# CTPLab/Tera-MIND

Hardware: AMD Instinct MI355X
Metric: denoising steps/sec on 64x64x(2 stains x 2 z) patches (interior patch-steps/s) (higher is better)
Workload: dtype f32; 1 GPU; configs[1]: b=32 images x 1 interior 64x64 patch (P=1, 128 padded + 32 collage patches/step), rna_slc=4, rna_num=229, stain=all, DDPM T=50 schedule, f32, mode A (pad+patchify -> UNet -> DDPM update); parallelism=dp1 (independent patch batches)

## Files before the change

tera-mind_amd/csrc/tm_kernels.hip:

```cpp
#include "tm_conv_pair.h"

#include <stdlib.h>
#include <string.h>

#include <type_traits>

namespace tmk {

template <int NZI, int WM, int TW, bool UPS = false>
struct C3Geo {
  static constexpr int TW_ = TW;
  static constexpr int MV = 4 * WM * 32;
  static constexpr int TR = (MV / TW < TW) ? (MV / TW) : TW;
  static constexpr int NPB = MV / (TR * TW);
  static constexpr int HR = TR + 2, HC = TW + 2;
  static constexpr int XV = NPB * NZI * HR * HC;
  static constexpr int XPIECES = XV * 2;
  static constexpr int PX = (XPIECES + 255) / 256;
  static constexpr int TZ = UPS ? 4 : 9;
  static constexpr int NTAP = TZ * NZI;
  static constexpr int WFLOATS = NTAP * 512;
  static constexpr int WPIECES = WFLOATS / 4;
  static constexpr int PW = (WPIECES + 255) / 256;
  static constexpr int TAPS_TOTAL = (NZI == 1) ? 9 : 3 * TZ;
// ... 518 lines not shown
  const f32x4 zero4 = {0.f, 0.f, 0.f, 0.f};
  auto load_x = [&](int cb) {
    const float* xp = a.x + (long)cb * a.x_plane;
#pragma unroll
    for (int z = 0; z < 2; ++z) {
      const float* b = xp + xoff + z * zplane;
      xr[z][0] = okl ? *(const f32x4*)(b - 8) : zero4;
      xr[z][1] = xoff >= 0 ? *(const f32x4*)(b) : zero4;
      xr[z][2] = xoff >= 0 ? *(const f32x4*)(b + 8) : zero4;
      xr[z][3] = okr ? *(const f32x4*)(b + 16) : zero4;
    }
  };
  auto put_t = [&](int p, const f32x4& d0, const f32x4& d1, const f32x4& d2, const f32x4& d3) __attribute__((always_inline)) {
    float* d = lds + xw + p * 4 * G::XP * 8;
    *(f32x4*)(d) = d0 - d2;
    *(f32x4*)(d + G::XP * 8) = d1 + d2;
    *(f32x4*)(d + 2 * G::XP * 8) = d2 - d1;
    *(f32x4*)(d + 3 * G::XP * 8) = d1 - d3;
  };

  load_x(0);
#pragma unroll
  for (int k = 0; k < G::KP; ++k) issue_piece(0, k);
  auto stage = [&](int cb, auto more_c) __attribute__((always_inline)) {
    constexpr bool more = decltype(more_c)::value;
    asm volatile("s_waitcnt vmcnt(0)" ::: "memory");
    __builtin_amdgcn_s_barrier();
    asm volatile("" ::: "memory");
    if (tid < G::XITEMS) {
      put_t(2, xr[0][0], xr[0][1], xr[0][2], xr[0][3]);
#pragma unroll
      for (int c = 0; c < 4; ++c) xr[0][c] = xr[0][c] + xr[1][c];
      put_t(0, xr[0][0], xr[0][1], xr[0][2], xr[0][3]);
      put_t(1, xr[1][0], xr[1][1], xr[1][2], xr[1][3]);
    }
    __builtin_amdgcn_s_waitcnt(0xC07F);
    asm volatile("" ::: "memory");
    __builtin_amdgcn_s_barrier();
    asm volatile("" ::: "memory");
    __builtin_amdgcn_sched_barrier(0);
    if (more) load_x(cb + 1);

    __builtin_amdgcn_s_setprio(1);
#pragma unroll
    for (int p = 0; p < 3; ++p) {
      const int n = cb * 3 + p;
      if (p > 0) {
        asm volatile("s_waitcnt vmcnt(0)" ::: "memory");
        __builtin_amdgcn_sched_barrier(0);
        __builtin_amdgcn_s_barrier();
        asm volatile("" ::: "memory");
        __builtin_amdgcn_sched_barrier(0);
      }
      const float* lwc = lw + (n & 1) * G::WSLOT + wb;
#pragma unroll
      for (int ky = 0; ky < 3; ++ky) {
#pragma unroll
        for (int q = 0; q < G::NQ; ++q) {
          const int tap = ky * 4 + q;
          const f32x4 wf = *(const f32x4*)(lwc + tap * 512);
          const f32x4 xf = ((const f32x4*)lds)[xb + xp_xtap<G>(p, q, ky) / 4];
#pragma unroll
          for (int kk = 0; kk < 4; ++kk) acc[p][q] = __builtin_amdgcn_mfma_f32_32x32x2f32(wf[kk], xf[kk], acc[p][q], 0, 0, 0);
          if (ky * G::NQ + q < G::KP && (p < 2 || more)) issue_piece(n + 1, ky * G::NQ + q);
        }
      }
    }
    __builtin_amdgcn_s_setprio(0);
  };
  for (int cb = 0; cb + 1 < a.Cbi; ++cb) stage(cb, std::true_type{});
  stage(a.Cbi - 1, std::false_type{});
  const int nte = 2 * nt + ch;
  if constexpr (HALF) {
    const int qh = __builtin_amdgcn_readfirstlane(wv >> 1);
    __syncthreads();
    auto hand_over = [&](const f32x16& t, int p) __attribute__((always_inline)) {
#pragma unroll
      for (int i = 0; i < 4; ++i) {
        const f32x4 v = {t[4 * i], t[4 * i + 1], t[4 * i + 2], t[4 * i + 3]};
        *(f32x4*)(lds + ((wv * 3 + p) * 4 + i) * 256 + lane * 4) = v;
      }
    };
    if (qh) {
#pragma unroll
      for (int p = 0; p < 3; ++p) hand_over(acc[p][0], p);
    } else {
#pragma unroll
      for (int p = 0; p < 3; ++p) hand_over(acc[p][1], p);
    }
    __syncthreads();
    f32x16 got[3];
#pragma unroll
    for (int p = 0; p < 3; ++p)
#pragma unroll
      for (int i = 0; i < 4; ++i) {
        const f32x4 v = *(const f32x4*)(lds + (((wv ^ 2) * 3 + p) * 4 + i) * 256 + lane * 4);
#pragma unroll
        for (int e = 0; e < 4; ++e) got[p][4 * i + e] = v[e];
      }
#pragma unroll
    for (int p = 0; p < 3; ++p) {
      acc[p][0] = qh ? (got[p] - acc[p][0]) - acc[p][1] : (acc[p][0] + acc[p][1]) + got[p];
      asm volatile("" : "+v"(acc[p][0]));
    }
#pragma unroll
    for (int z = 0; z < 2; ++z) {
      f32x16 o[1][1];
      o[0][0] = acc[0][0] + acc[1 + z][0];
      asm volatile("" : "+v"(o[0][0]));
      const int ooff[1] = {ooff0 >= 0 ? ooff0 + (z * S * S + qh) * 8 : -1};
      __builtin_amdgcn_sched_barrier(0);
      conv_epilogue<1, 1>(a, o, nte, h, on, ooff, 2 * S);
    }
  } else {
#pragma unroll
    for (int p = 0; p < 3; ++p) {
      const f32x16 ev = (acc[p][0] + acc[p][1]) + acc[p][2];
      acc[p][1] = (acc[p][1] - acc[p][2]) - acc[p][3];
      acc[p][0] = ev;
      asm volatile("" : "+v"(acc[p][0]), "+v"(acc[p][1]));
    }
#pragma unroll
    for (int z = 0; z < 2; ++z)
#pragma unroll
      for (int par = 0; par < 2; ++par) {
        f32x16 o[1][1];
        o[0][0] = acc[0][par] + acc[1 + z][par];
        asm volatile("" : "+v"(o[0][0]));
        const int ooff[1] = {ooff0 >= 0 ? ooff0 + (z * S * S + par) * 8 : -1};
        __builtin_amdgcn_sched_barrier(0);
        conv_epilogue<1, 1>(a, o, nte, h, on, ooff, 2 * S);
      }
  }
}

template <int HALF, int TW, int PIPE = 0>
struct XQGeo {
  static constexpr int TW_ = TW;
  static constexpr int NW = HALF ? 4 : 8;
  static constexpr int MG = 16 * NW;
  static constexpr int GW = TW / 4;
  static constexpr int TR = (MG / GW < TW) ? (MG / GW) : TW;
  static constexpr int NPB = MG / (TR * GW);
  static constexpr int HR = TR + 2;
  static constexpr int XP = NPB * HR * GW;
  static constexpr int XITEMS = XP * 2;
  static_assert(XP % 8 == 0, "whole groups of eight staging items (tm_conv_frag.h)");
  static constexpr int WTAP = 256;
  static constexpr int WSLOT = 18 * WTAP;
  static constexpr int KP = (18 + NW - 1) / NW;
  static constexpr int XSET = 6 * XP * 8;
  static constexpr int NSET = PIPE ? 2 : 3;
  static constexpr int XCH = NW * 3 * 1024;
  static constexpr int LDS_BYTES = (2 * WSLOT + NSET * XSET > XCH ? 2 * WSLOT + NSET * XSET : XCH) * 4;
  static_assert(2 * WSLOT * 4 <= 65536 && LDS_BYTES <= 160 * 1024, "LDS-DMA destinations below 64 KiB, the CU's LDS");
  static_assert(!PIPE || !HALF || LDS_BYTES <= 80 * 1024, "two workgroups of the small tile per CU");
};
template <class V>
TM_HD V xq_transform(int q, const V (&d)[6]) {
  switch (q) {
    case 0: return (4.f * d[0] - 5.f * d[2]) + d[4];
    case 1: return (d[3] + d[4]) - 4.f * (d[1] + d[2]);
    case 2: return 4.f * (d[1] - d[2]) - (d[3] - d[4]);
    case 3: return 2.f * (d[3] - d[1]) + (d[4] - d[2]);
    case 4: return 2.f * (d[1] - d[3]) + (d[4] - d[2]);
    default: return (4.f * d[1] - 5.f * d[3]) + d[5];
  }
}
TM_HD constexpr int xq_lane_group(int tw, int i32) { return tw == 8 ? conv_lane_voxel(16, i32) : i32; }
template <class G>
TM_HD constexpr int xq_xtap(int q, int ky) { return q * G::XP * 8 + conv_frag_off(ky * G::GW, 0, G::XP); }
template <class G>
TM_HD constexpr int xq_xfrag(int set, int qh, int lxb) { return set * G::XSET + 3 * qh * G::XP * 8 + lxb; }
template <class G>
TM_HD constexpr int xq_xstage(int set, int q, int item) {
  return set * G::XSET + q * G::XP * 8 + conv_frag_off(conv_stage_row(item), conv_stage_half(item), G::XP);
}

template <int HALF, int TW, int PIPE>
__global__ __launch_bounds__(HALF ? 256 : 512, 2) void conv3d_xquad(ConvArgs a) {
  using G = XQGeo<HALF, TW, PIPE>;
  static_assert(G::XITEMS <= 64 * G::NW, "one staging item per thread");
  extern __shared__ __attribute__((aligned(16))) float lds[];
  float* lw = lds;

  const int tid = threadIdx.x;
  const int lane = tid & 63, wv = tid >> 6;
  const int i32 = lane & 31, h = lane >> 5;

  const int S = a.S;
  const ConvTile t = conv_tile_of<TW, G::TR, false, false>(a);
  const int nt = t.nt, pg = t.pg, tr = t.tr, tc = t.tc;

  long xoff = -1;
  bool okl = false, okr = false;
  if (tid < G::XITEMS) {
    const int half = conv_stage_half(tid);
    int v = conv_stage_row(tid);
    const int j = v % G::GW; v /= G::GW;
    const int hr = v % G::HR;
    const int ps = v / G::HR;
    const int n = pg * G::NPB + ps;
    const int y = tr * G::TR + hr - 1, x = tc * TW + 4 * j;
    if (n < a.N && y >= 0 && y < S) {
      xoff = (long)n * a.x_nstride + ((long)y * S + x) * 8 + half * 4;
      okl = x > 0;
      okr = x + 4 < S;
    }
  }
  const long zplane = (long)S * S * 8;
  int xw = 2 * G::WSLOT + xq_xstage<G>(0, 0, tid);
  asm volatile("" : "+v"(xw));

  const int gt = wv >> 1;
  const int qh = wv & 1;
  int xb[3], on[1], ooff0;
  {
    const ConvLane l = conv_lane_of<G::TR, G::GW, G::HR * G::GW, G::GW, G::XP>(gt * 32 + xq_lane_group(TW, i32), h, 0, 0);
#pragma unroll
    for (int p = 0; p < 3; ++p) {
      xb[p] = (2 * G::WSLOT + xq_xfrag<G>(p, qh, l.xb)) / 4;
      asm volatile("" : "+v"(xb[p]));
    }
    const int n = pg * G::NPB + l.ps;
    on[0] = n;
    const int y = tr * G::TR + l.r, x = tc * TW + 4 * l.c;
    ooff0 = n < a.N ? (y * S + x) * 8 : -1;
  }
  const int wb = 3 * qh * G::WTAP + conv_frag_off(i32, h, 32);

  f32x16 acc[3][3];
  clear_acc(acc);

  const unsigned lw_lds = (unsigned)(size_t)(__attribute__((address_space(3))) float*)lw;
  const rsrc_words wrs = weight_rsrc<true>(a.w + (long)nt * a.Cbi * 3 * G::WSLOT, a.Cbi * 3 * G::WSLOT * 4);
  const int wvo = lane * 16;
  const int wvu = __builtin_amdgcn_readfirstlane(wv);
  auto issue_piece = [&](int n, int k) __attribute__((always_inline)) {
    lds_dma_piece<4, 18, G::NW>(lw_lds, (n & 1) * G::WSLOT, n * G::WSLOT, k, wvu, wvo, wrs);
  };

  f32x4 xr[2][6];
  const f32x4 zero4 = {0.f, 0.f, 0.f, 0.f};
  auto load_x = [&](int cb) {
    const float* xp = a.x + (long)cb * a.x_plane;
#pragma unroll
    for (int z = 0; z < 2; ++z) {
      const float* b = xp + xoff + z * zplane;
      xr[z][0] = okl ? *(const f32x4*)(b - 8) : zero4;
#pragma unroll
      for (int c = 0; c < 4; ++c) xr[z][1 + c] = xoff >= 0 ? *(const f32x4*)(b + 8 * c) : zero4;
      xr[z][5] = okr ? *(const f32x4*)(b + 32) : zero4;
    }
  };
  auto put_t = [&](int p, const f32x4 (&d)[6]) __attribute__((always_inline)) {
    float* o = lds + xw + p * G::XSET;
#pragma unroll
    for (int q = 0; q < 6; ++q) *(f32x4*)(o + q * G::XP * 8) = xq_transform(q, d);
  };

  if constexpr (PIPE) {
  const bool stg = tid < G::XITEMS;
  const bool ldw = __builtin_amdgcn_readfirstlane(wv * 64 < G::XITEMS);
  auto load_xc = [&](int cb) __attribute__((always_inline)) {
    const float* xp = a.x + (long)cb * a.x_plane + (xoff >= 0 ? xoff : 0);
#pragma unroll
    for (int z = 0; z < 2; ++z) {
      const float* b = xp + z * zplane;
      xr[z][0] = *(const f32x4*)(okl ? b - 8 : b);
#pragma unroll
      for (int c = 0; c < 4; ++c) xr[z][1 + c] = *(const f32x4*)(b + 8 * c);
      xr[z][5] = *(const f32x4*)(okr ? b + 32 : b);
    }
  };
  auto mask_x = [&](int z) __attribute__((always_inline)) {
    xr[z][0] = okl ? xr[z][0] : zero4;
#pragma unroll
    for (int c = 0; c < 4; ++c) xr[z][1 + c] = xoff >= 0 ? xr[z][1 + c] : zero4;
    xr[z][5] = okr ? xr[z][5] : zero4;
#pragma unroll
    for (int c = 0; c < 6; ++c) asm volatile("" : "+v"(xr[z][c]));
  };
  int xw4 = xw / 4;
  asm volatile("" : "+v"(xw4));
  auto put_q = [&](int q, const f32x4 (&d)[6], int set) __attribute__((always_inline)) {
    ((f32x4*)lds)[xw4 + set * (G::XSET / 4) + q * G::XP * 2] = xq_transform(q, d);
  };
  constexpr int LOADTAP = G::KP > 3 ? G::KP - 1 : 2;
  static_assert(LOADTAP < 9, "inside the product");

#pragma unroll
  for (int k = 0; k < G::KP; ++k) lds_dma_piece<4, 18, G::NW>(lw_lds, 0, 2 * G::WSLOT, k, wvu, wvo, wrs);
  if (ldw) load_xc(0);
  else {
#pragma unroll
    for (int c = 0; c < 12; ++c) xr[c / 6][c % 6] = zero4;
  }
  mask_x(0);
  if (stg) {
#pragma unroll
    for (int q = 0; q < 6; ++q) put_q(q, xr[0], 0);
  }
  auto block = [&](int cb, auto more_c) __attribute__((always_inline)) {
    constexpr bool more = decltype(more_c)::value;
    __builtin_amdgcn_s_setprio(1);
#pragma unroll
    for (int i = 0; i < 3; ++i) {
      const int n = cb * 3 + i, par = n & 1;
      const int p = 2 - i;
      const bool follows = i < 2 || more;
      if (i == 2 && more && ldw) asm volatile("s_waitcnt vmcnt(12)" ::: "memory");
      else asm volatile("s_waitcnt vmcnt(0)" ::: "memory");
      __builtin_amdgcn_s_waitcnt(0xC07F);
      __builtin_amdgcn_sched_barrier(0);
      __builtin_amdgcn_s_barrier();
      asm volatile("" ::: "memory");
      __builtin_amdgcn_sched_barrier(0);
      const float* lwc = lw + par * G::WSLOT + wb;
      const int xbn = xb[0] + par * (G::XSET / 4);
      const int nsrc = (i == 2 ? cb * 3 + 5 : cb * 3 + p - 1) * G::WSLOT;
#pragma unroll
      for (int ky = 0; ky < 3; ++ky) {
#pragma unroll
        for (int q = 0; q < 3; ++q) {
          const int tap = ky * 3 + q;
          const f32x4 wf = *(const f32x4*)(lwc + (ky * 6 + q) * G::WTAP);
          const f32x4 xf = ((const f32x4*)lds)[xbn + xq_xtap<G>(q, ky) / 4];
          if (follows) {
            if (tap == 0 && i != 1) mask_x(i == 0 ? 1 : 0);
            if (i == 1) {
              if (tap == 0) {
#pragma unroll
                for (int c = 0; c < 6; ++c) xr[0][c] = xr[0][c] + xr[1][c];
              }
              if (tap < 3 && stg) { put_q(2 * tap, xr[0], par ^ 1); put_q(2 * tap + 1, xr[0], par ^ 1); }
            } else if (tap < 6 && stg) {
              put_q(tap, i == 0 ? xr[1] : xr[0], par ^ 1);
            }
            if (tap < G::KP) lds_dma_piece<4, 18, G::NW>(lw_lds, (par ^ 1) * G::WSLOT, nsrc, tap, wvu, wvo, wrs);
            if (i == 1 && more && tap == LOADTAP && ldw) load_xc(cb + 1);
          }
#pragma unroll
          for (int kk = 0; kk < 4; ++kk) acc[p][q] = __builtin_amdgcn_mfma_f32_32x32x2f32(wf[kk], xf[kk], acc[p][q], 0, 0, 0);
        }
      }
    }
    __builtin_amdgcn_s_setprio(0);
  };
  for (int cb = 0; cb + 1 < a.Cbi; ++cb) block(cb, std::true_type{});
  block(a.Cbi - 1, std::false_type{});
  } else {
  load_x(0);
#pragma unroll
  for (int k = 0; k < G::KP; ++k) issue_piece(0, k);
  auto stage = [&](int cb, auto more_c) __attribute__((always_inline)) {
    constexpr bool more = decltype(more_c)::value;
    asm volatile("s_waitcnt vmcnt(0)" ::: "memory");
    __builtin_amdgcn_s_barrier();
    asm volatile("" ::: "memory");
    if (tid < G::XITEMS) {
      put_t(2, xr[0]);
#pragma unroll
      for (int c = 0; c < 6; ++c) xr[0][c] = xr[0][c] + xr[1][c];
      put_t(0, xr[0]);
      put_t(1, xr[1]);
    }
    __builtin_amdgcn_s_waitcnt(0xC07F);
    asm volatile("" ::: "memory");
    __builtin_amdgcn_s_barrier();
    asm volatile("" ::: "memory");
    __builtin_amdgcn_sched_barrier(0);
    if (more) load_x(cb + 1);

    __builtin_amdgcn_s_setprio(1);
#pragma unroll
    for (int p = 0; p < 3; ++p) {
      const int n = cb * 3 + p;
      if (p > 0) {
        asm volatile("s_waitcnt vmcnt(0)" ::: "memory");
        __builtin_amdgcn_sched_barrier(0);
        __builtin_amdgcn_s_barrier();
        asm volatile("" ::: "memory");
        __builtin_amdgcn_sched_barrier(0);
      }
      const float* lwc = lw + (n & 1) * G::WSLOT + wb;
#pragma unroll
      for (int ky = 0; ky < 3; ++ky) {
#pragma unroll
        for (int q = 0; q < 3; ++q) {
          const f32x4 wf = *(const f32x4*)(lwc + (ky * 6 + q) * G::WTAP);
          const f32x4 xf = ((const f32x4*)lds)[xb[p] + xq_xtap<G>(q, ky) / 4];
#pragma unroll
          for (int kk = 0; kk < 4; ++kk) acc[p][q] = __builtin_amdgcn_mfma_f32_32x32x2f32(wf[kk], xf[kk], acc[p][q], 0, 0, 0);
          if (ky * 3 + q < G::KP && (p < 2 || more)) issue_piece(n + 1, ky * 3 + q);
        }
      }
    }
    __builtin_amdgcn_s_setprio(0);
  };
  for (int cb = 0; cb + 1 < a.Cbi; ++cb) stage(cb, std::true_type{});
  stage(a.Cbi - 1, std::false_type{});
  }

  const int qhu = __builtin_amdgcn_readfirstlane(qh);
#pragma unroll
  for (int p = 0; p < 3; ++p) {
    if (qhu) {
      const f32x16 sp = acc[p][0] + acc[p][1];
      acc[p][0] = acc[p][0] - acc[p][1];
      acc[p][1] = sp;
    } else {
      const f32x16 s = acc[p][1] + acc[p][2];
      acc[p][2] = acc[p][1] - acc[p][2];
      acc[p][1] = s;
    }
    asm volatile("" : "+v"(acc[p][0]), "+v"(acc[p][1]), "+v"(acc[p][2]));
  }
  __syncthreads();
#pragma unroll
  for (int p = 0; p < 3; ++p)
#pragma unroll
    for (int i = 0; i < 4; ++i) {
      const f32x16& tl = qhu ? acc[p][1] : acc[p][2];
      const f32x4 v = {tl[4 * i], tl[4 * i + 1], tl[4 * i + 2], tl[4 * i + 3]};
      *(f32x4*)(lds + ((wv * 3 + p) * 4 + i) * 256 + lane * 4) = v;
    }
  __syncthreads();
  f32x16 got[3];
#pragma unroll
  for (int p = 0; p < 3; ++p)
#pragma unroll
    for (int i = 0; i < 4; ++i) {
      const f32x4 v = *(const f32x4*)(lds + (((wv ^ 1) * 3 + p) * 4 + i) * 256 + lane * 4);
#pragma unroll
      for (int e = 0; e < 4; ++e) got[p][4 * i + e] = v[e];
    }
#pragma unroll
  for (int p = 0; p < 3; ++p) {
    f32x16 c0, c1;
    if (qhu) {
      c0 = got[p] + 2.f * acc[p][0];
      c1 = (got[p] + 8.f * acc[p][0]) + acc[p][2];
    } else {
      c0 = (acc[p][0] + acc[p][1]) + got[p];
      c1 = acc[p][1] + 4.f * got[p];
    }
    acc[p][0] = c0;
    acc[p][1] = c1;
    asm volatile("" : "+v"(acc[p][0]), "+v"(acc[p][1]));
  }
#pragma unroll
  for (int z = 0; z < 2; ++z)
#pragma unroll
    for (int par = 0; par < 2; ++par) {
      f32x16 o[1][1];
      o[0][0] = acc[0][par] + acc[1 + z][par];
      asm volatile("" : "+v"(o[0][0]));
      const int ooff[1] = {ooff0 >= 0 ? ooff0 + (z * S * S + 2 * par + qh) * 8 : -1};
      __builtin_amdgcn_sched_barrier(0);
      conv_epilogue<1, 1>(a, o, nt, h, on, ooff, 2 * S);
    }
}

template <int WM, int WN>
__global__ __launch_bounds__(256, 2) void conv1_mfma(ConvArgs a) {
  constexpr int MV = 4 * WM * 32;
  constexpr int KC = 4;
  constexpr int XP = KC * MV * 2 / 256;
  constexpr int NT64 = WN / 2;
  constexpr int WP = NT64 * KC * 64 * 2 / 256;
  __shared__ __attribute__((aligned(16))) float lds[NT64 * KC * 512 + KC * MV * 8];
  float* lw = lds;
  float* lx = lds + NT64 * KC * 512;

  const int tid = threadIdx.x;
  const int lane = tid & 63, wv = tid >> 6;
  const int i32 = lane & 31, h = lane >> 5;
  const int bid = xcd_swizzle(blockIdx.x, gridDim.x);
  const int nt = bid % a.ntile;
  const int mtile = bid / a.ntile;
  const long VPN = (long)a.Z * a.S * a.S;
  const long vtot = VPN * a.N;

  long xoff[XP];
  int xkc[XP];
#pragma unroll
  for (int k = 0; k < XP; ++k) {
    const int i = tid + k * 256;
    const int half = i & 1;
    const int v = (i >> 1) % MV;
    xkc[k] = (i >> 1) / MV;
    const long vg = (long)mtile * MV + v;
    long off = -1;
    if (vg < vtot) {
      const long n = vg / VPN;
      off = n * a.x_nstride + (vg - n * VPN) * 8 + half * 4;
    }
    xoff[k] = off;
  }
  const float* wsrc = a.w + (long)nt * NT64 * a.Cbi * 512;

  int xb[WM], on[WM], ooff[WM];
#pragma unroll
  for (int mt = 0; mt < WM; ++mt) {
    const int v = (wv * WM + mt) * 32 + i32;
    xb[mt] = v * 8 + 4 * h;
    const long vg = (long)mtile * MV + v;
    if (vg < vtot) {
      const long n = vg / VPN;
      on[mt] = (int)n;
      ooff[mt] = (int)((vg - n * VPN) * 8);
    } else { on[mt] = 0; ooff[mt] = -1; }
  }
  const int wb = i32 * 8 + 4 * h;

  f32x16 acc[WN][WM];
#pragma unroll
  for (int ct = 0; ct < WN; ++ct)
#pragma unroll
    for (int mt = 0; mt < WM; ++mt)
#pragma unroll
      for (int r = 0; r < 16; ++r) acc[ct][mt][r] = 0.f;

  f32x4 xr[XP], wr[WP];
  const f32x4 zero4 = {0.f, 0.f, 0.f, 0.f};
  auto load_stage = [&](int cb0) {
#pragma unroll
    for (int k = 0; k < XP; ++k) {
      const int cb = cb0 + xkc[k];
      xr[k] = (xoff[k] >= 0 && cb < a.Cbi) ? *(const f32x4*)(a.x + (long)cb * a.x_plane + xoff[k]) : zero4;
    }
#pragma unroll
    for (int k = 0; k < WP; ++k) {
      const int i = tid + k * 256;
      const int t64 = i / (KC * 128), j = i - t64 * (KC * 128);
      const int cb = cb0 + j / 128;
      wr[k] = (cb < a.Cbi) ? *(const f32x4*)(wsrc + ((long)t64 * a.Cbi + cb0) * 512 + j * 4) : zero4;
    }
  };

  load_stage(0);
  for (int cb0 = 0; cb0 < a.Cbi; cb0 += KC) {
    __syncthreads();
#pragma unroll
    for (int k = 0; k < XP; ++k) *(f32x4*)(lx + (tid + k * 256) * 4) = xr[k];
#pragma unroll
    for (int k = 0; k < WP; ++k) *(f32x4*)(lw + (tid + k * 256) * 4) = wr[k];
    __syncthreads();
    if (cb0 + KC < a.Cbi) load_stage(cb0 + KC);
#pragma unroll
    for (int kc = 0; kc < KC; ++kc) {
      f32x4 wf[WN], xf[WM];
#pragma unroll
      for (int ct = 0; ct < WN; ++ct) wf[ct] = *(const f32x4*)(lw + (ct >> 1) * (KC * 512) + kc * 512 + (ct & 1) * 256 + wb);
#pragma unroll
      for (int mt = 0; mt < WM; ++mt) xf[mt] = *(const f32x4*)(lx + kc * MV * 8 + xb[mt]);
#pragma unroll
      for (int kk = 0; kk < 4; ++kk)
#pragma unroll
        for (int ct = 0; ct < WN; ++ct)
#pragma unroll
          for (int mt = 0; mt < WM; ++mt)
            acc[ct][mt] = __builtin_amdgcn_mfma_f32_32x32x2f32(wf[ct][kk], xf[mt][kk], acc[ct][mt], 0, 0, 0);
    }
  }
  conv_epilogue<WM, WN>(a, acc, nt, h, on, ooff, 0);
}

static bool conv_fills_chip(long vox, long tiles) { return (vox / 256) * tiles >= 512; }

int conv1_form(long vox, int ntile, int tile_variant) {
  if (tile_variant == 3) return (ntile & 1) == 0 ? 3 : 0;
  const int variant = tile_variant ? tile_variant : (conv_fills_chip(vox, ntile) ? 2 : 1);
  if (variant == 2 && (ntile & 1) == 0 && conv_fills_chip(vox, ntile / 2)) return 3;
  return variant == 2 ? 2 : 1;
}

int conv_tile(int form, long ovox, int ntile, int S, int tile_variant) {
  if (S == 4) return 1;
  if (form == CF_XQUAD) return tile_variant ? (tile_variant == 2 ? 2 : 1) : ((ovox / 1024) * 2 * ntile >= 256 ? 2 : 1);
  const long tiles = (form == CF_ZSKIP_UPS || form == CF_PAIR_UPS) ? 4L * ntile : ntile;
  const int variant = tile_variant ? tile_variant : (conv_fills_chip(ovox, tiles) ? 2 : 1);
  return variant == 2 ? 2 : 1;
}

static bool xquad_pipe_default(bool half, int tw) {
  static const bool on = [] {
    const char* v = getenv("TM_CONV_XQUAD_PIPE");
    return !(v && atoi(v) == 0);
  }();
  return on && !half && tw == 16;
}

template <void (*KERN)(ConvArgs), class G, int BLOCK = 256>
static hipError_t launch_tiled(const ConvArgs& a, long factor, hipStream_t s) {
  static DevOnce attr_once;
  if (attr_once.need()) {
    hipError_t e = hipFuncSetAttribute((const void*)KERN, hipFuncAttributeMaxDynamicSharedMemorySize, G::LDS_BYTES);
    if (e != hipSuccess) return e;
    attr_once.mark();
  }
  const long tiles = (long)(a.S / G::TW_) * (a.S / G::TR);
  const long pgs = (a.N + G::NPB - 1) / G::NPB;
  hipLaunchKernelGGL(KERN, dim3((unsigned)(pgs * tiles * factor * a.ntile)), dim3(BLOCK), G::LDS_BYTES, s, a);
  return hipGetLastError();
}
template <int MAXTW, class F>
static hipError_t with_tile_width(int S, F f) {
  if constexpr (MAXTW >= 32)
    if (S >= 32) return f(std::integral_constant<int, 32>{});
  if (S >= 16) return f(std::integral_constant<int, 16>{});
  return f(std::integral_constant<int, 8>{});
}
template <int NZI, bool UPS>
static hipError_t launch_c3(const ConvArgs& a, bool large, hipStream_t s) {
  const long factor = UPS ? 4L * a.Z : a.Z;
  if (a.S == 4) return launch_tiled<conv3d_mfma<NZI, 1, 4, UPS>, C3Geo<NZI, 1, 4, UPS>>(a, factor, s);
  return with_tile_width<32>(a.S, [&](auto tw) {
    constexpr int TW = decltype(tw)::value;
    return large ? launch_tiled<conv3d_mfma<NZI, 2, TW, UPS>, C3Geo<NZI, 2, TW, UPS>>(a, factor, s)
                 : launch_tiled<conv3d_mfma<NZI, 1, TW, UPS>, C3Geo<NZI, 1, TW, UPS>>(a, factor, s);
  });
}

hipError_t launch_conv_mfma(const ConvLaunch& L, hipStream_t s) {
  ConvArgs a;
  a.x = L.x.p; a.x_nstride = L.x.nstride; a.x_plane = L.x.plane();
  a.w = L.w.w; a.bias = L.w.bias;
  a.y = L.y.p; a.y_nstride = L.y.nstride; a.y_plane = L.y.plane(); a.Cob = L.y.Cb;
  a.res = L.res ? L.res->p : nullptr; a.res_nstride = L.res ? L.res->nstride : 0;
  a.gate = L.gate ? L.gate->p : nullptr; a.gate_nstride = L.gate ? L.gate->nstride : 0;
  const int form = L.w.form;
  if (L.w.taps != conv_form_taps(form)) return hipErrorInvalidValue;
  if (L.gate_half) {
    int ls = 0;
    while ((1 << ls) < L.y.H) ++ls;
    if (!L.gate || form != CF_1X1 || (1 << ls) != L.y.H || L.y.H != L.y.W || ls < 1) return hipErrorInvalidValue;
    a.gate_ls = ls;
  }
  a.N = L.x.N; a.S = L.x.H; a.Z = L.x.Z; a.Cbi = L.w.Cbi; a.ntile = L.w.ntile; a.flags = L.flags;
  if (L.x.Cb != L.w.Cbi || L.x.H != L.x.W) return hipErrorInvalidValue;
  if (L.fuse_norm) {
    if (form != CF_PAIR || L.zmode != ZM_PAD1 || L.x.Z != 2 || L.w.Cout != 64 || L.w.ntile != 1 || L.res || L.gate || L.flags ||
        !L.norm_w || !L.mod_scale || !L.mod_shift || L.per_image < 1)
      return hipErrorInvalidValue;
    if (conv_tile(form, (long)L.x.N * 2 * L.x.H * L.x.H, 1, L.x.H, L.tile_variant) != 2) return hipErrorInvalidValue;
    if (!L.a2.p || L.a2.Cb != 8 || L.a2.N != L.x.N || L.a2.Z != 2 || L.a2.H != L.x.H || L.a2.W != L.x.H) return hipErrorInvalidValue;
    if (L.y.Cb != 8 || L.y.Z != 2 || L.y.H != L.x.H) return hipErrorInvalidValue;
    a.y = L.a2.p; a.y_nstride = L.a2.nstride; a.y_plane = L.a2.plane();
    a.norm_w = L.norm_w; a.mod_scale = L.mod_scale; a.mod_shift = L.mod_shift; a.mod_stride = L.mod_stride;
    a.per_image = L.per_image; a.inv_c = L.inv_c;
  }
  if (L.y.Cb > L.w.ntile * 8 || L.y.N != L.x.N) return hipErrorInvalidValue;
  const long vox = (long)a.N * a.Z * a.S * a.S;
  if (form == CF_1X1) {
    if (L.flags & EPI_UP2) return hipErrorInvalidValue;
    if (L.y.H != L.x.H || L.y.Z != L.x.Z) return hipErrorInvalidValue;
    const int form1 = conv1_form(vox, a.ntile, L.tile_variant);
    if (form1 == 3) {
      const long mt = (vox + 255) / 256;
      a.ntile /= 2;
      hipLaunchKernelGGL((conv1_mfma<2, 4>), dim3((unsigned)(mt * a.ntile)), dim3(256), 0, s, a);
    } else if (form1 == 2) {
      const long mt = (vox + 255) / 256;
      hipLaunchKernelGGL((conv1_mfma<2, 2>), dim3((unsigned)(mt * a.ntile)), dim3(256), 0, s, a);
    } else if (form1 == 1) {
      const long mt = (vox + 127) / 128;
      hipLaunchKernelGGL((conv1_mfma<1, 2>), dim3((unsigned)(mt * a.ntile)), dim3(256), 0, s, a);
    } else return hipErrorInvalidValue;
    return hipGetLastError();
  }
  const int S = a.S;
  const bool z2 = L.x.Z == 2 && L.y.Z == 2, up2 = (L.flags & EPI_UP2) != 0;
  a.Zin = L.x.Z; a.zoff = 0;
  switch (form) {
    case CF_INPLANE:
      if (L.zmode == ZM_PAD1 ? (L.x.Z != 1 || L.y.Z != 1) : (L.zmode != ZM_INPLANE || L.y.Z != L.x.Z)) return hipErrorInvalidValue;
      break;
    case CF_PLANES3:
      if (L.zmode == ZM_PAD1 ? (L.y.Z != L.x.Z || L.x.Z == 2) : (L.zmode != ZM_VALID || L.y.Z != L.x.Z - 2)) return hipErrorInvalidValue;
      if (L.zmode == ZM_PAD1) a.zoff = -1;
      break;
    case CF_ZSKIP: case CF_PAIR:
      if (L.zmode != ZM_PAD1 || !z2) return hipErrorInvalidValue;
      break;
    case CF_XPAIR: case CF_XQUAD:
      if (L.zmode != ZM_PAD1 || !z2 || L.x.H < 8 || up2) return hipErrorInvalidValue;
      break;
    case CF_ZSKIP_UPS: case CF_PAIR_UPS:
      if (L.zmode != ZM_UPS || !z2 || up2 || L.res || L.gate) return hipErrorInvalidValue;
      break;
    default: return hipErrorInvalidValue;
  }
  a.Z = L.y.Z;
  if (S != 4 && S != 8 && S != 16 && S != 32 && S != 64 && S != 128) return hipErrorInvalidValue;
  if ((up2 || L.zmode == ZM_UPS) ? (L.y.H != 2 * S) : (L.y.H != S)) return hipErrorInvalidValue;
  if (L.res_half) {
    int ls = 0;
    while ((1 << ls) < L.y.H) ++ls;
    if (!L.res || (1 << ls) != L.y.H || L.y.H != L.y.W || ls < 1 || up2) return hipErrorInvalidValue;
    a.res_ls = ls;
  }
  const bool large = conv_tile(form, (long)a.N * a.Z * a.S * a.S, a.ntile, S, L.tile_variant) == 2;
  switch (form) {
    case CF_INPLANE: return launch_c3<1, false>(a, large, s);
    case CF_PLANES3: return launch_c3<3, false>(a, large, s);
    case CF_ZSKIP: return launch_c3<2, false>(a, large, s);
    case CF_ZSKIP_UPS: return launch_c3<2, true>(a, large, s);
    case CF_PAIR:
      if (S == 4) return launch_tiled<conv3d_zpair<1, 4, false>, ZPGeo<1, 4>>(a, 1, s);
      return with_tile_width<32>(S, [&](auto tw) {
        constexpr int TW = decltype(tw)::value;
        if (L.fuse_norm) return launch_tiled<conv3d_zpair<0, TW, true>, ZPGeo<0, TW>>(a, 1, s);
        return large ? launch_tiled<conv3d_zpair<0, TW, false>, ZPGeo<0, TW>>(a, 1, s)
                     : launch_tiled<conv3d_zpair<1, TW, false>, ZPGeo<1, TW>>(a, 1, s);
      });
    case CF_PAIR_UPS:
      if (S == 4) return launch_tiled<conv3d_zpair_ups<1, 4>, ZPUGeo<1, 4>>(a, 4, s);
      return with_tile_width<32>(S, [&](auto tw) {
        constexpr int TW = decltype(tw)::value;
        return large ? launch_tiled<conv3d_zpair_ups<0, TW>, ZPUGeo<0, TW>>(a, 4, s)
                     : launch_tiled<conv3d_zpair_ups<1, TW>, ZPUGeo<1, TW>>(a, 4, s);
      });
    case CF_XQUAD:
      a.ntile = (L.w.Cout + 31) / 32;
      if (L.xquad_sched < -1 || L.xquad_sched > 1) return hipErrorInvalidValue;
      return with_tile_width<16>(S, [&](auto tw) {
        constexpr int TW = decltype(tw)::value;
        if (L.xquad_sched < 0 ? xquad_pipe_default(!large, TW) : L.xquad_sched == 1)
          return large ? launch_tiled<conv3d_xquad<0, TW, 1>, XQGeo<0, TW, 1>, 64 * XQGeo<0, TW, 1>::NW>(a, 1, s)
                       : launch_tiled<conv3d_xquad<1, TW, 1>, XQGeo<1, TW, 1>, 64 * XQGeo<1, TW, 1>::NW>(a, 1, s);
        return large ? launch_tiled<conv3d_xquad<0, TW, 0>, XQGeo<0, TW, 0>, 64 * XQGeo<0, TW, 0>::NW>(a, 1, s)
                     : launch_tiled<conv3d_xquad<1, TW, 0>, XQGeo<1, TW, 0>, 64 * XQGeo<1, TW, 0>::NW>(a, 1, s);
      });
    default:
      return with_tile_width<16>(S, [&](auto tw) {
        constexpr int TW = decltype(tw)::value;
        return large ? launch_tiled<conv3d_xpair<0, TW>, XPGeo<0, TW>, 64 * XPGeo<0, TW>::NW>(a, 1, s)
                     : launch_tiled<conv3d_xpair<1, TW>, XPGeo<1, TW>, 64 * XPGeo<1, TW>::NW>(a, 1, s);
      });
  }
}

template <class G, int HALF, int TW, bool UPS>
static int zpair_frag_addrs(int what, int wv, int p, int ky, int kx, int sub, int* out) {
  constexpr int NC = HALF ? 1 : 2, KW = UPS ? 2 : 3;
  constexpr int lx = G::LDS_BYTES / 4 - 3 * G::XV * 8;
  if (p < 0 || p > 2) return -1;
  if (what == 2 ? (ky < 0 || ky >= G::PX) : (ky < 0 || ky >= KW || kx < 0 || kx >= KW)) return -1;
  if (what == 0 ? (sub < 0 || sub >= NC) : what == 1 ? (sub < 0 || sub > (UPS ? 3 : 0)) : false) return -1;
  const int vt = HALF ? (wv & 1) : wv, ct0 = HALF ? (wv >> 1) : 0;
  for (int lane = 0; lane < 64; ++lane) {
    const int i32 = lane & 31, h = lane >> 5;
    int a = -1;
    if (what == 0) a = zp_wtap(UPS ? p * 4 + ky * 2 + kx : p * 9 + ky * 3 + kx, sub) + conv_w_off(ct0 * 32 + i32, 4 * h);
    else if (what == 1)
      a = lx + zp_xtap<G>(p, ky, kx) + conv_lane_of<G::TR, TW, G::PS, G::HC, G::XV>(vt * 32 + conv_lane_voxel(TW, i32), h, sub >> 1, sub & 1).xb;
    else {
      const int i = wv * 64 + lane + ky * 256;
      if (conv_stage_row(i) < G::XV) a = lx + p * G::XV * 8 + conv_frag_off(conv_stage_row(i), conv_stage_half(i), G::XV);
    }
    out[lane] = a < 0 ? -1 : a * 4;
  }
  return 0;
}
template <int HALF, int TW>
static int xpair_frag_addrs(int what, int wv, int p, int ky, int q, int* out) {
  using G = XPGeo<HALF, TW>;
  if (p < 0 || p > 2 || q < 0 || q >= (what == 2 ? 4 : G::NQ) || ky < 0 || ky > (what == 2 ? 0 : 2)) return -1;
  const int pt = HALF ? 0 : (wv >> 1), ch = wv & 1, q0 = HALF ? (wv >> 1) * 2 : 0;
  for (int lane = 0; lane < 64; ++lane) {
    const int i32 = lane & 31, h = lane >> 5, tid = wv * 64 + lane;
    int a = -1;
    if (what == 0) a = q0 * 512 + conv_w_off(ch * 32 + i32, 4 * h) + (ky * 4 + q) * 512;
    else if (what == 1)
      a = 2 * G::WSLOT + q0 * G::XP * 8 + conv_lane_of<G::TR, G::PWD, G::HR * G::PWD, G::PWD, G::XP>(pt * 32 + i32, h, 0, 0).xb + xp_xtap<G>(p, q, ky);
    else if (tid < G::XITEMS)
      a = 2 * G::WSLOT + conv_frag_off(conv_stage_row(tid), conv_stage_half(tid), G::XP) + (p * 4 + q) * G::XP * 8;
    out[lane] = a < 0 ? -1 : a * 4;
  }
  return 0;
}
template <int HALF, int TW, int PIPE>
static int xquad_frag_addrs(int what, int wv, int p, int ky, int q, int set, int* out) {
  using G = XQGeo<HALF, TW, PIPE>;
  if (wv >= G::NW || p < 0 || p > 2 || q < 0 || q >= (what == 2 ? 6 : 3) || ky < 0 || ky > (what == 2 ? 0 : 2)) return -1;
  if (set < 0 || set >= G::NSET) return -1;
  const int gt = wv >> 1, qh = wv & 1;
  for (int lane = 0; lane < 64; ++lane) {
    const int i32 = lane & 31, h = lane >> 5, tid = wv * 64 + lane;
    int a = -1;
    if (what == 0) a = 3 * qh * G::WTAP + conv_frag_off(i32, h, 32) + (ky * 6 + q) * G::WTAP;
    else if (what == 1)
      a = 2 * G::WSLOT + xq_xtap<G>(q, ky) +
          xq_xfrag<G>(set, qh, conv_lane_of<G::TR, G::GW, G::HR * G::GW, G::GW, G::XP>(gt * 32 + xq_lane_group(TW, i32), h, 0, 0).xb);
    else if (tid < G::XITEMS)
      a = 2 * G::WSLOT + xq_xstage<G>(set, q, tid);
    out[lane] = a < 0 ? -1 : a * 4;
  }
  return 0;
}
int conv_xquad_lds_bytes(int half, int tw, int sched) {
  if (half < 0 || half > 1 || (tw != 8 && tw != 16) || sched < 0 || sched > 1) return -1;
  if (sched) return half ? (tw == 8 ? XQGeo<1, 8, 1>::LDS_BYTES : XQGeo<1, 16, 1>::LDS_BYTES) : (tw == 8 ? XQGeo<0, 8, 1>::LDS_BYTES : XQGeo<0, 16, 1>::LDS_BYTES);
  return half ? (tw == 8 ? XQGeo<1, 8, 0>::LDS_BYTES : XQGeo<1, 16, 0>::LDS_BYTES) : (tw == 8 ? XQGeo<0, 8, 0>::LDS_BYTES : XQGeo<0, 16, 0>::LDS_BYTES);
}
int conv_frag_addrs(int kernel, int half, int tw, int what, int wv, int p, int ky, int kx, int sub, int* out) {
  const bool xq = kernel == 4 || kernel == 5;
  if (!out || kernel < 0 || kernel > 5 || kernel == 3 || half < 0 || half > 1 || what < 0 || what > 2 || wv < 0 || wv > (xq ? 7 : 3)) return -1;
  if (kernel == 4 && tw == 8) return half ? xquad_frag_addrs<1, 8, 0>(what, wv, p, ky, kx, p, out) : xquad_frag_addrs<0, 8, 0>(what, wv, p, ky, kx, p, out);
  if (kernel == 4 && tw == 16) return half ? xquad_frag_addrs<1, 16, 0>(what, wv, p, ky, kx, p, out) : xquad_frag_addrs<0, 16, 0>(what, wv, p, ky, kx, p, out);
  if (kernel == 5 && what == 0 && sub != 0) return -1;
  if (kernel == 5 && tw == 8) return half ? xquad_frag_addrs<1, 8, 1>(what, wv, p, ky, kx, sub, out) : xquad_frag_addrs<0, 8, 1>(what, wv, p, ky, kx, sub, out);
  if (kernel == 5 && tw == 16) return half ? xquad_frag_addrs<1, 16, 1>(what, wv, p, ky, kx, sub, out) : xquad_frag_addrs<0, 16, 1>(what, wv, p, ky, kx, sub, out);
  if (xq) return -1;
#define TM_FRAG(H, T)                                                                                              \
  if (half == H && tw == T) {                                                                                      \
    if (kernel == 0) return zpair_frag_addrs<ZPGeo<H, T>, H, T, false>(what, wv, p, ky, kx, sub, out);              \
    if (kernel == 1) return zpair_frag_addrs<ZPUGeo<H, T>, H, T, true>(what, wv, p, ky, kx, sub, out);              \
  }
  TM_FRAG(1, 4) TM_FRAG(0, 8) TM_FRAG(1, 8) TM_FRAG(0, 16) TM_FRAG(1, 16) TM_FRAG(0, 32) TM_FRAG(1, 32)
#undef TM_FRAG
  if (kernel == 2 && tw == 8) return half ? xpair_frag_addrs<1, 8>(what, wv, p, ky, kx, out) : xpair_frag_addrs<0, 8>(what, wv, p, ky, kx, out);
  if (kernel == 2 && tw == 16) return half ? xpair_frag_addrs<1, 16>(what, wv, p, ky, kx, out) : xpair_frag_addrs<0, 16>(what, wv, p, ky, kx, out);
  return -1;
}

struct PrepArgs { PrepLaunch L; };
struct PrepDropArgs { PrepLaunch L; DropRng r; };
__device__ __forceinline__ DropRng rng_of(const PrepArgs&) { return DropRng{0ull, 0u, 0u}; }
__device__ __forceinline__ DropRng rng_of(const PrepDropArgs& a) { return a.r; }

__device__ __forceinline__ float sumsq8(const f32x4& a0, const f32x4& a1) {
  return a0[0] * a0[0] + a0[1] * a0[1] + a0[2] * a0[2] + a0[3] * a0[3] + a1[0] * a1[0] + a1[1] * a1[1] + a1[2] * a1[2] + a1[3] * a1[3];
}
template <int NSUB, bool CACHED, bool DRAW = false, class Args = PrepArgs, int WV = 4, int NCW = 8>
__global__ __launch_bounds__(WV * 64) void prep_kernel(Args pa) {
  constexpr bool WIDE = WV > 4;
  static_assert(!WIDE || (NSUB == 1 && CACHED && !DRAW && WV * NCW >= 4), "the wide form is a cached NSUB 1 form");
  const PrepLaunch& L = pa.L;
  const DropRng R = rng_of(pa);
  __shared__ float red[4][NSUB][64];
  const int tid = threadIdx.x, lane = tid & 63, wv = WIDE ? __builtin_amdgcn_readfirstlane(tid >> 6) : tid >> 6;
  const int S = L.S, Z = L.Z;
  const long vpn = (long)Z * S * S;
  const long vidx = (long)blockIdx.x * 64 + lane;
  const bool valid = vidx < vpn * L.N;
  int n = 0, z = 0, y = 0, x = 0;
  if (valid) {
    n = (int)(vidx / vpn);
    int rem = (int)(vidx - (long)n * vpn);
    z = rem / (S * S); rem -= z * S * S;
    y = rem / S; x = rem - y * S;
  }
  long soff[3][NSUB];
  long splane[3];
#pragma unroll
  for (int k = 0; k < 3; ++k) {
    if (k >= L.nsrc) { splane[k] = 0; continue; }
    int Ss = S;
    if (L.resample == RS_UP2) Ss = S / 2;
    if (L.resample == RS_DOWN2 || L.resample == RS_PICK2) Ss = S * 2;
    splane[k] = (long)Z * Ss * Ss * 8;
#pragma unroll
    for (int sub = 0; sub < NSUB; ++sub) {
      int ns = n, ys = y, xs = x;
      if (L.resample == RS_UP2) { ys = y >> 1; xs = x >> 1; }
      if (L.resample == RS_DOWN2) { ys = 2 * y + (sub >> 1); xs = 2 * x + (sub & 1); }
      if (L.resample == RS_PICK2) { ys = 2 * y; xs = 2 * x; }
      if (L.src[k].collage) {
        const int q1 = L.p1 - 1, q2 = L.p2 - 1;
        const int bi = n / (q1 * q2);
        const int q = n - bi * q1 * q2;
        int i = q / q2, j = q - i * q2;
        ys += Ss / 2; if (ys >= Ss) { ys -= Ss; i += 1; }
        xs += Ss / 2; if (xs >= Ss) { xs -= Ss; j += 1; }
        ns = bi * L.p1 * L.p2 + i * L.p2 + j;
      }
      soff[k][sub] = (long)ns * L.src[k].nstride + ((long)(z * Ss + ys) * Ss + xs) * 8;
    }
  }
  const int cb0 = L.src[0].Cb, cb01 = cb0 + ((L.nsrc > 1) ? L.src[1].Cb : 0);
// ... 918 lines not shown
```

Baseline: 1011 interior patch-steps/s.

## Interleave Winograd staging and DMA between individual MFMAs with double-buffered fragments

Restructures the pipelined XQ conv inner loop so each tap's four MFMAs are separated by scheduling barriers. LDS fragment loads for the next tap, weight DMA pieces and input-transform stores are placed between those MFMAs, so memory work overlaps matrix math instead of being grouped together. Lanes that do not stage are redirected to a spare LDS scratch region so they can execute the stores without branching. The loader path becomes a compile-time template parameter, giving separate specialisations for loading and non-loading waves. This costs extra LDS for the spare region and adds register pressure from double-buffered fragments, and the forced ordering may block useful compiler scheduling.

New measurement: 1016 interior patch-steps/s, median of 6. About the same (+0.4%).

```diff
diff --git a/tera-mind_amd/csrc/tm_kernels.hip b/tera-mind_amd/csrc/tm_kernels.hip
--- a/tera-mind_amd/csrc/tm_kernels.hip
+++ b/tera-mind_amd/csrc/tm_kernels.hip
@@ -694,7 +694,8 @@
   static constexpr int XSET = 6 * XP * 8;
   static constexpr int NSET = PIPE ? 2 : 3;
   static constexpr int XCH = NW * 3 * 1024;
-  static constexpr int LDS_BYTES = (2 * WSLOT + NSET * XSET > XCH ? 2 * WSLOT + NSET * XSET : XCH) * 4;
+  static constexpr int SPARE = PIPE && XITEMS % 64 ? 5 * XP * 8 + 64 * 4 : 0;
+  static constexpr int LDS_BYTES = (2 * WSLOT + NSET * XSET + SPARE > XCH ? 2 * WSLOT + NSET * XSET + SPARE : XCH) * 4;
   static_assert(2 * WSLOT * 4 <= 65536 && LDS_BYTES <= 160 * 1024, "LDS-DMA destinations below 64 KiB, the CU's LDS");
   static_assert(!PIPE || !HALF || LDS_BYTES <= 80 * 1024, "two workgroups of the small tile per CU");
 };
@@ -825,8 +826,9 @@
   };
   int xw4 = xw / 4;
   asm volatile("" : "+v"(xw4));
-  auto put_q = [&](int q, const f32x4 (&d)[6], int set) __attribute__((always_inline)) {
-    ((f32x4*)lds)[xw4 + set * (G::XSET / 4) + q * G::XP * 2] = xq_transform(q, d);
+  const int xsp = (2 * G::WSLOT + G::NSET * G::XSET) / 4 + lane;
+  auto put_q = [&](int q, const f32x4 (&d)[6], int base) __attribute__((always_inline)) {
+    ((f32x4*)lds)[base + q * G::XP * 2] = xq_transform(q, d);
   };
   constexpr int LOADTAP = G::KP > 3 ? G::KP - 1 : 2;
   static_assert(LOADTAP < 9, "inside the product");
@@ -841,56 +843,87 @@
   mask_x(0);
   if (stg) {
 #pragma unroll
-    for (int q = 0; q < 6; ++q) put_q(q, xr[0], 0);
-  }
-  auto block = [&](int cb, auto more_c) __attribute__((always_inline)) {
+    for (int q = 0; q < 6; ++q) put_q(q, xr[0], xw4);
+  }
+  auto block = [&](int cb, auto more_c, auto stg_c) __attribute__((always_inline)) {
     constexpr bool more = decltype(more_c)::value;
+    constexpr bool STG = decltype(stg_c)::value;
     __builtin_amdgcn_s_setprio(1);
 #pragma unroll
     for (int i = 0; i < 3; ++i) {
       const int n = cb * 3 + i, par = n & 1;
       const int p = 2 - i;
       const bool follows = i < 2 || more;
-      if (i == 2 && more && ldw) asm volatile("s_waitcnt vmcnt(12)" ::: "memory");
+      const float* lwc = lw + par * G::WSLOT + wb;
+      int xbn = xb[0] + par * (G::XSET / 4);
+      int xws = xw4 + (par ^ 1) * (G::XSET / 4);
+      if (G::SPARE) xws = stg ? xws : xsp;
+      asm volatile("" : "+v"(xbn), "+v"(xws));
+      const int nsrc = (i == 2 ? cb * 3 + 5 : cb * 3 + p - 1) * G::WSLOT;
+      if (i == 2 && more && STG) asm volatile("s_waitcnt vmcnt(12)" ::: "memory");
       else asm volatile("s_waitcnt vmcnt(0)" ::: "memory");
       __builtin_amdgcn_s_waitcnt(0xC07F);
       __builtin_amdgcn_sched_barrier(0);
       __builtin_amdgcn_s_barrier();
       asm volatile("" ::: "memory");
       __builtin_amdgcn_sched_barrier(0);
-      const float* lwc = lw + par * G::WSLOT + wb;
-      const int xbn = xb[0] + par * (G::XSET / 4);
-      const int nsrc = (i == 2 ? cb * 3 + 5 : cb * 3 + p - 1) * G::WSLOT;
-#pragma unroll
-      for (int ky = 0; ky < 3; ++ky) {
-#pragma unroll
-        for (int q = 0; q < 3; ++q) {
-          const int tap = ky * 3 + q;
-          const f32x4 wf = *(const f32x4*)(lwc + (ky * 6 + q) * G::WTAP);
-          const f32x4 xf = ((const f32x4*)lds)[xbn + xq_xtap<G>(q, ky) / 4];
-          if (follows) {
-            if (tap == 0 && i != 1) mask_x(i == 0 ? 1 : 0);
-            if (i == 1) {
-              if (tap == 0) {
-#pragma unroll
-                for (int c = 0; c < 6; ++c) xr[0][c] = xr[0][c] + xr[1][c];
-              }
-              if (tap < 3 && stg) { put_q(2 * tap, xr[0], par ^ 1); put_q(2 * tap + 1, xr[0], par ^ 1); }
-            } else if (tap < 6 && stg) {
-              put_q(tap, i == 0 ? xr[1] : xr[0], par ^ 1);
-            }
-            if (tap < G::KP) lds_dma_piece<4, 18, G::NW>(lw_lds, (par ^ 1) * G::WSLOT, nsrc, tap, wvu, wvo, wrs);
-            if (i == 1 && more && tap == LOADTAP && ldw) load_xc(cb + 1);
+      f32x4 wf[2], xf[2];
+      auto frags = [&](int tap) __attribute__((always_inline)) {
+        const int ky = tap / 3, q = tap % 3;
+        wf[tap & 1] = *(const f32x4*)(lwc + (ky * 6 + q) * G::WTAP);
+        xf[tap & 1] = ((const f32x4*)lds)[xbn + xq_xtap<G>(q, ky) / 4];
+      };
+      frags(0);
+#pragma unroll
+      for (int tap = 0; tap < 9; ++tap) {
+        const int q = tap % 3, b = tap & 1;
+        const bool st = STG && follows;
+        __builtin_amdgcn_sched_barrier(0);
+        acc[p][q] = __builtin_amdgcn_mfma_f32_32x32x2f32(wf[b][0], xf[b][0], acc[p][q], 0, 0, 0);
+        __builtin_amdgcn_sched_barrier(0);
+        if (follows && tap < G::KP) lds_dma_piece<4, 18, G::NW>(lw_lds, (par ^ 1) * G::WSLOT, nsrc, tap, wvu, wvo, wrs);
+        if (tap < 8) frags(tap + 1);
+        __builtin_amdgcn_sched_barrier(0);
+        if (st) {
+          if (i == 1) {
+            if (tap == 0) {
+#pragma unroll
+              for (int c = 0; c < 6; ++c) xr[0][c] = xr[0][c] + xr[1][c];
+            } else if (tap < 3) put_q(2 * tap, xr[0], xws);
+          } else {
+            if (tap == 0) mask_x(i == 0 ? 1 : 0);
+            else if (tap < 6) put_q(tap, i == 0 ? xr[1] : xr[0], xws);
           }
-#pragma unroll
-          for (int kk = 0; kk < 4; ++kk) acc[p][q] = __builtin_amdgcn_mfma_f32_32x32x2f32(wf[kk], xf[kk], acc[p][q], 0, 0, 0);
         }
+        __builtin_amdgcn_sched_barrier(0);
+        acc[p][q] = __builtin_amdgcn_mfma_f32_32x32x2f32(wf[b][1], xf[b][1], acc[p][q], 0, 0, 0);
+        __builtin_amdgcn_sched_barrier(0);
+        if (st) {
+          if (i == 1) {
+            if (tap == 0) put_q(0, xr[0], xws);
+            else if (tap < 3) put_q(2 * tap + 1, xr[0], xws);
+          } else if (tap == 0) put_q(0, i == 0 ? xr[1] : xr[0], xws);
+        }
+        __builtin_amdgcn_sched_barrier(0);
+        acc[p][q] = __builtin_amdgcn_mfma_f32_32x32x2f32(wf[b][2], xf[b][2], acc[p][q], 0, 0, 0);
+        __builtin_amdgcn_sched_barrier(0);
+        if (st && i == 1) {
+          if (tap == 0) put_q(1, xr[0], xws);
+          if (more && tap == LOADTAP) load_xc(cb + 1);
+        }
+        __builtin_amdgcn_sched_barrier(0);
+        acc[p][q] = __builtin_amdgcn_mfma_f32_32x32x2f32(wf[b][3], xf[b][3], acc[p][q], 0, 0, 0);
       }
     }
     __builtin_amdgcn_s_setprio(0);
   };
-  for (int cb = 0; cb + 1 < a.Cbi; ++cb) block(cb, std::true_type{});
-  block(a.Cbi - 1, std::false_type{});
+  if (ldw) {
+    for (int cb = 0; cb + 1 < a.Cbi; ++cb) block(cb, std::true_type{}, std::true_type{});
+    block(a.Cbi - 1, std::false_type{}, std::true_type{});
+  } else {
+    for (int cb = 0; cb + 1 < a.Cbi; ++cb) block(cb, std::true_type{}, std::false_type{});
+    block(a.Cbi - 1, std::false_type{}, std::false_type{});
+  }
   } else {
   load_x(0);
 #pragma unroll
```

## Inline xquad epilogue with early residual/bias loads and retune tile selection

Applied to the files above, without the earlier changes.

Replaces the generic per-slice conv_epilogue call in the xquad Winograd-style kernel with an inlined epilogue. Bias and residual loads are issued early, overlapping the LDS exchange and the barriers, and the barriers use raw s_barrier with explicit waitcnt. Accumulator roles are permuted so the LDS-exchanged tile is always acc[p][2], which removes a per-lane select. The tile heuristic also switches to the half tile and the pipelined schedule at S>=64 with many workgroups, and gated layers are now rejected for xquad. The cost is higher register pressure from holding 16 residual vectors, plus hand-written waitcnt and barrier code that is fragile.

After: 1015 interior patch-steps/s before, 1038 interior patch-steps/s after, median of 6. +2.2%, better.

```diff
diff --git a/tera-mind_amd/csrc/tm_kernels.hip b/tera-mind_amd/csrc/tm_kernels.hip
--- a/tera-mind_amd/csrc/tm_kernels.hip
+++ b/tera-mind_amd/csrc/tm_kernels.hip
@@ -945,12 +945,35 @@
   }
 
   const int qhu = __builtin_amdgcn_readfirstlane(qh);
+  const bool okv = ooff0 >= 0;
+  const long yl = okv ? (long)on[0] * a.y_nstride + ooff0 + qh * 8 + 4 * h : 0;
+  const long rl = okv ? (long)on[0] * a.res_nstride + (a.res_ls ? half_res_off(ooff0, a.res_ls) : ooff0 + qh * 8) + 4 * h : 0;
+  const long rplane = a.res_ls ? a.y_plane >> 2 : a.y_plane;
+  const int rz = a.res_ls ? S * S * 2 : S * S * 8, rp = a.res_ls ? 8 : 16;
+  const float* rsrc = a.res ? a.res : a.bias;
+  f32x4 bv[4], rv[2][2][4];
+#pragma unroll
+  for (int g = 0; g < 4; ++g) {
+    const int cob = nt * 4 + g;
+    bv[g] = *(const f32x4*)(a.bias + (long)(cob < a.Cob ? cob : 0) * 8 + 4 * h);
+  }
+  auto load_res = [&](int z, int par) __attribute__((always_inline)) {
+#pragma unroll
+    for (int g = 0; g < 4; ++g) {
+      const int cob = nt * 4 + g;
+      const long uni = (long)cob * rplane + z * rz + par * rp;
+      rv[z][par][g] = *(const f32x4*)(rsrc + (cob < a.Cob && okv && a.res ? rl + uni : 0));
+    }
+  };
+  load_res(0, 0);
+  load_res(0, 1);
 #pragma unroll
   for (int p = 0; p < 3; ++p) {
     if (qhu) {
       const f32x16 sp = acc[p][0] + acc[p][1];
       acc[p][0] = acc[p][0] - acc[p][1];
-      acc[p][1] = sp;
+      acc[p][1] = acc[p][2];
+      acc[p][2] = sp;
     } else {
       const f32x16 s = acc[p][1] + acc[p][2];
       acc[p][2] = acc[p][1] - acc[p][2];
@@ -958,16 +981,25 @@
     }
     asm volatile("" : "+v"(acc[p][0]), "+v"(acc[p][1]), "+v"(acc[p][2]));
   }
-  __syncthreads();
+  __builtin_amdgcn_sched_barrier(0);
+  __builtin_amdgcn_s_barrier();
+  asm volatile("" ::: "memory");
+  __builtin_amdgcn_sched_barrier(0);
 #pragma unroll
   for (int p = 0; p < 3; ++p)
 #pragma unroll
     for (int i = 0; i < 4; ++i) {
-      const f32x16& tl = qhu ? acc[p][1] : acc[p][2];
+      const f32x16& tl = acc[p][2];
       const f32x4 v = {tl[4 * i], tl[4 * i + 1], tl[4 * i + 2], tl[4 * i + 3]};
       *(f32x4*)(lds + ((wv * 3 + p) * 4 + i) * 256 + lane * 4) = v;
     }
-  __syncthreads();
+  load_res(1, 0);
+  asm volatile("" ::: "memory");
+  __builtin_amdgcn_s_waitcnt(0xC07F);
+  __builtin_amdgcn_sched_barrier(0);
+  __builtin_amdgcn_s_barrier();
+  asm volatile("" ::: "memory");
+  __builtin_amdgcn_sched_barrier(0);
   f32x16 got[3];
 #pragma unroll
   for (int p = 0; p < 3; ++p)
@@ -982,7 +1014,7 @@
     f32x16 c0, c1;
     if (qhu) {
       c0 = got[p] + 2.f * acc[p][0];
-      c1 = (got[p] + 8.f * acc[p][0]) + acc[p][2];
+      c1 = (got[p] + 8.f * acc[p][0]) + acc[p][1];
     } else {
       c0 = (acc[p][0] + acc[p][1]) + got[p];
       c1 = acc[p][1] + 4.f * got[p];
@@ -991,17 +1023,39 @@
     acc[p][1] = c1;
     asm volatile("" : "+v"(acc[p][0]), "+v"(acc[p][1]));
   }
+  load_res(1, 1);
 #pragma unroll
   for (int z = 0; z < 2; ++z)
 #pragma unroll
     for (int par = 0; par < 2; ++par) {
-      f32x16 o[1][1];
-      o[0][0] = acc[0][par] + acc[1 + z][par];
-      asm volatile("" : "+v"(o[0][0]));
-      const int ooff[1] = {ooff0 >= 0 ? ooff0 + (z * S * S + 2 * par + qh) * 8 : -1};
-      __builtin_amdgcn_sched_barrier(0);
-      conv_epilogue<1, 1>(a, o, nt, h, on, ooff, 2 * S);
-    }
+      f32x16 o = acc[0][par] + acc[1 + z][par];
+      asm volatile("" : "+v"(o));
+#pragma unroll
+      for (int g = 0; g < 4; ++g) {
+        f32x4 v;
+        v[0] = o[4 * g + 0] + bv[g][0];
+        v[1] = o[4 * g + 1] + bv[g][1];
+        v[2] = o[4 * g + 2] + bv[g][2];
+        v[3] = o[4 * g + 3] + bv[g][3];
+        if (a.flags & EPI_GELU) {
+#pragma unroll
+          for (int j = 0; j < 4; ++j) v[j] = gelu_tanh_hw(v[j]);
+        }
+        if (a.res) v = rv[z][par][g] + v;
+        rv[z][par][g] = v;
+        asm volatile("" : "+v"(rv[z][par][g]));
+      }
+    }
+#pragma unroll
+  for (int z = 0; z < 2; ++z)
+#pragma unroll
+    for (int par = 0; par < 2; ++par)
+#pragma unroll
+      for (int g = 0; g < 4; ++g) {
+        const int cob = nt * 4 + g;
+        const long uni = (long)cob * a.y_plane + z * (S * S * 8) + par * 16;
+        if (cob < a.Cob && okv) *(f32x4*)(a.y + yl + uni) = rv[z][par][g];
+      }
 }
 
 template <int WM, int WN>
@@ -1118,20 +1172,24 @@
   return variant == 2 ? 2 : 1;
 }
 
+static long xquad_large_wgs(long ovox, int ntile) { return (ovox / 1024) * 2 * ntile; }
+static bool xquad_many_wgs(long ovox, int ntile, int S) { return S >= 64 && xquad_large_wgs(ovox, ntile) >= 2048; }
+
 int conv_tile(int form, long ovox, int ntile, int S, int tile_variant) {
   if (S == 4) return 1;
-  if (form == CF_XQUAD) return tile_variant ? (tile_variant == 2 ? 2 : 1) : ((ovox / 1024) * 2 * ntile >= 256 ? 2 : 1);
+  if (form == CF_XQUAD)
+    return tile_variant ? (tile_variant == 2 ? 2 : 1) : (xquad_large_wgs(ovox, ntile) >= 256 && !xquad_many_wgs(ovox, ntile, S) ? 2 : 1);
   const long tiles = (form == CF_ZSKIP_UPS || form == CF_PAIR_UPS) ? 4L * ntile : ntile;
   const int variant = tile_variant ? tile_variant : (conv_fills_chip(ovox, tiles) ? 2 : 1);
   return variant == 2 ? 2 : 1;
 }
 
-static bool xquad_pipe_default(bool half, int tw) {
+static bool xquad_pipe_default(bool half, int tw, bool many) {
   static const bool on = [] {
     const char* v = getenv("TM_CONV_XQUAD_PIPE");
     return !(v && atoi(v) == 0);
   }();
-  return on && !half && tw == 16;
+  return on && tw == 16 && (!half || many);
 }
 
 template <void (*KERN)(ConvArgs), class G, int BLOCK = 256>
@@ -1228,6 +1286,7 @@
       break;
     case CF_XPAIR: case CF_XQUAD:
       if (L.zmode != ZM_PAD1 || !z2 || L.x.H < 8 || up2) return hipErrorInvalidValue;
+      if (form == CF_XQUAD && L.gate) return hipErrorInvalidValue;
       break;
     case CF_ZSKIP_UPS: case CF_PAIR_UPS:
       if (L.zmode != ZM_UPS || !z2 || up2 || L.res || L.gate) return hipErrorInvalidValue;
@@ -1269,7 +1328,7 @@
       if (L.xquad_sched < -1 || L.xquad_sched > 1) return hipErrorInvalidValue;
       return with_tile_width<16>(S, [&](auto tw) {
         constexpr int TW = decltype(tw)::value;
-        if (L.xquad_sched < 0 ? xquad_pipe_default(!large, TW) : L.xquad_sched == 1)
+        if (L.xquad_sched < 0 ? xquad_pipe_default(!large, TW, xquad_many_wgs((long)a.N * a.Z * a.S * a.S, L.w.ntile, S)) : L.xquad_sched == 1)
           return large ? launch_tiled<conv3d_xquad<0, TW, 1>, XQGeo<0, TW, 1>, 64 * XQGeo<0, TW, 1>::NW>(a, 1, s)
                        : launch_tiled<conv3d_xquad<1, TW, 1>, XQGeo<1, TW, 1>, 64 * XQGeo<1, TW, 1>::NW>(a, 1, s);
         return large ? launch_tiled<conv3d_xquad<0, TW, 0>, XQGeo<0, TW, 0>, 64 * XQGeo<0, TW, 0>::NW>(a, 1, s)
```
